# Acly/dlimgedit

Hardware: AMD Instinct MI355X
Metric: images/sec encode+mask @1024x1024 (higher is better)
Workload: dtype f16; 1 GPU; SAM vit_b encoder + 1 point prompt, 1 image(s)/GPU/step, 1024x1024 RGBA, inputs and masks resident in HBM; timed through the extension entry point dlimg_amd_encode_and_mask (device pointers in and out) -- the drop-in table itself, host buffers in and out, is `abi_path`; weights=seeded synthetic, lanes_per_gpu=4, lanes_fed_by_the_step_queue=3, requests_coalesced_per_pass=4, passes_queued_per_lane=2

## Files before the change

dlimgedit_amd/csrc/kernels/attention_window.hip:

```cpp
#include "device_common.hpp"
#include "kernels.hpp"

#include <algorithm>
#include <cstdio>
#include <cstdlib>
#include <mutex>
#include <string>
#include <vector>

namespace dlimg {
namespace {

constexpr int WS = 14;
constexpr int SLOTS = 224;
constexpr int NW = 5;
constexpr int GRID = 64;
constexpr int V_STRIDE = 96;
constexpr int G_STRIDE = 33;
typedef short short4_t __attribute__((ext_vector_type(4)));
typedef __attribute__((address_space(3))) short4_t lds_short4_t;

struct WinSlot { int token; bool dummy; bool pad; };

DLIMG_DEVICE WinSlot win_slot(int slot, int wy, int wx) {
    int ty = slot >> 4, tx = slot & 15;
    int gy = wy * WS + ty, gx = wx * WS + tx;
    WinSlot s;
    s.dummy = tx >= WS;
    s.pad = !s.dummy && (gy >= GRID || gx >= GRID);
    s.token = gy * GRID + gx;
    return s;
}

DLIMG_DEVICE int k_row(int slot) { const int tx = slot & 15; return (slot >> 4) * WS + (tx < WS ? tx : WS - 1); }

template <int HD>
__global__ __launch_bounds__(448, 4) void attention_window_kernel(const half_t* __restrict__ qkv,
                                                               const half_t* __restrict__ qkv_pad,
                                                               const half_t* __restrict__ rel_h,
                                                               const half_t* __restrict__ rel_w,
                                                               half_t* __restrict__ out, int heads,
                                                               unsigned long long* stamps_arg) {
#ifdef DLIMG_TUNING
    unsigned long long* const stamps = stamps_arg;
#else
    unsigned long long* const stamps = nullptr;
#endif
    unsigned long long tstamp[8] = {0, 0, 0, 0, 0, 0, 0, 0};
    auto stamp = [&](int i) { if (stamps) tstamp[i] = __builtin_amdgcn_s_memtime(); };
    stamp(0);
    constexpr int KS = HD / 16;
    constexpr int DT = (HD + 31) / 32;
    constexpr int K_STRIDE = HD + 8;
    constexpr int CHUNKS = HD / 8;
    static_assert(DT * 32 <= V_STRIDE, "head dimension tiles must fit the padded V row");

    extern __shared__ __attribute__((aligned(16))) char smem[];
    half_t* lds_k = reinterpret_cast<half_t*>(smem);
    half_t* lds_v = lds_k + WS * WS * K_STRIDE;
    float* lds_g = reinterpret_cast<float*>(smem);

    const int D = heads * HD;
    const int ld = 3 * D;
    const int head = blockIdx.x % heads;
    const int win = (blockIdx.x / heads) % (NW * NW);
    const int img = blockIdx.x / (heads * NW * NW);
    const int wy = win / NW, wx = win % NW;
    const half_t* base = qkv + (size_t)img * 4096 * ld;
    const int tid = threadIdx.x;
    const int lane = lane_id();
    const int wave = wave_id();
    const int hi = lane >> 5, l31 = lane & 31;

    const int token0 = wy * WS * GRID + wx * WS;
    const int qslot = wave * 32 + l31;
    const WinSlot qs = win_slot(qslot, wy, wx);
    const bool q_real = !qs.dummy && !qs.pad;
    half8_t qf[KS];
    {
        const half_t* qrow = base + (size_t)(q_real ? qs.token : token0) * ld + head * HD + hi * 8;
#pragma unroll
        for (int ks = 0; ks < KS; ++ks) qf[ks] = *reinterpret_cast<const half8_t*>(qrow + ks * 16);
    }
    half8_t rfh[KS], rfw[KS];
    {
        const int rrow = l31 < 2 * WS - 1 ? l31 : 2 * WS - 2;
#pragma unroll
        for (int ks = 0; ks < KS; ++ks) {
            rfh[ks] = *reinterpret_cast<const half8_t*>(rel_h + rrow * HD + ks * 16 + hi * 8);
            rfw[ks] = *reinterpret_cast<const half8_t*>(rel_w + rrow * HD + ks * 16 + hi * 8);
        }
    }
    static_assert((SLOTS * CHUNKS) % 448 == 0, "K/V chunks split evenly over the workgroup");
    constexpr int KV_IT = SLOTS * CHUNKS / 448;
#if defined(DLIMG_TUNING) && defined(DLIMG_WINDOW_KV_EARLY)
    constexpr int KV_EARLY = HD == 64 ? KV_IT : DLIMG_WINDOW_KV_EARLY;
#else
    constexpr int KV_EARLY = HD == 64 ? KV_IT : 3;
#endif
    half8_t kreg[KV_IT], vreg[KV_IT];
    auto request_kv = [&](int it) {
        const int idx = tid + it * 448;
        const WinSlot ws = win_slot(idx / CHUNKS, wy, wx);
        const half_t* row = (ws.pad ? qkv_pad : base + (size_t)(ws.dummy ? token0 : ws.token) * ld) + head * HD + (idx % CHUNKS) * 8;
        kreg[it] = *reinterpret_cast<const half8_t*>(row + D);
        vreg[it] = *reinterpret_cast<const half8_t*>(row + 2 * D);
    };
#pragma unroll
    for (int it = 0; it < KV_EARLY; ++it) request_kv(it);
    __builtin_amdgcn_sched_barrier(0);
    stamp(1);
#pragma unroll
    for (int ks = 0; ks < KS; ++ks) {
        if (!q_real) qf[ks] = zero_h8();
        if (l31 >= 2 * WS - 1) { rfh[ks] = zero_h8(); rfw[ks] = zero_h8(); }
    }

    float* g = lds_g + wave * 32 * G_STRIDE;
    const int ty_q = qslot >> 4, tx_q = qslot & 15;
    float bh[WS];
    float bw[8];
    {
        float16_t acc = zero16();
#pragma unroll
        for (int ks = 0; ks < KS; ++ks) acc = mfma32(rfh[ks], qf[ks], acc);
#pragma unroll
        for (int r = 0; r < 16; ++r) g[l31 * G_STRIDE + acc_row(r, hi)] = acc[r];
        __builtin_amdgcn_sched_barrier(0);
        float16_t acc_w = zero16();
#pragma unroll
        for (int ks = 0; ks < KS; ++ks) acc_w = mfma32(rfw[ks], qf[ks], acc_w);
        if (KV_EARLY < KV_IT) {
            __builtin_amdgcn_sched_barrier(0);
#pragma unroll
            for (int it = KV_EARLY; it < KV_IT; ++it) request_kv(it);
            __builtin_amdgcn_sched_barrier(0);
        }
        __builtin_amdgcn_fence(__ATOMIC_RELEASE, "wavefront");
        __builtin_amdgcn_wave_barrier();
#pragma unroll
        for (int ky = 0; ky < WS; ++ky) bh[ky] = g[l31 * G_STRIDE + ty_q + (WS - 1) - ky] * sqrtf((float)HD);
        __builtin_amdgcn_fence(__ATOMIC_RELEASE, "wavefront");
        __builtin_amdgcn_wave_barrier();
#pragma unroll
        for (int r = 0; r < 16; ++r) g[l31 * G_STRIDE + acc_row(r, hi)] = acc_w[r];
        __builtin_amdgcn_fence(__ATOMIC_RELEASE, "wavefront");
        __builtin_amdgcn_wave_barrier();
#pragma unroll
        for (int e = 0; e < 8; ++e) {
            const int tx = (e & 3) + 8 * (e >> 2) + 4 * hi;
            bw[e] = tx < WS ? g[l31 * G_STRIDE + tx_q + (WS - 1) - tx] * sqrtf((float)HD) : -INFINITY;
        }
        __syncthreads();
    }
    stamp(2);

#pragma unroll
    for (int it = 0; it < KV_IT; ++it) {
        const int idx = tid + it * 448;
        const int slot = idx / CHUNKS, ch = idx % CHUNKS;
        const bool dummy = (slot & 15) >= WS;
        if (!dummy) *reinterpret_cast<half8_t*>(lds_k + k_row(slot) * K_STRIDE + ch * 8) = kreg[it];
        *reinterpret_cast<half8_t*>(lds_v + slot * V_STRIDE + ch * 8) = dummy ? zero_h8() : vreg[it];
    }
    if (DT * 32 > HD) {
        constexpr int PADC = (DT * 32 - HD) / 8;
        for (int idx = tid; idx < SLOTS * PADC; idx += 448)
            *reinterpret_cast<half8_t*>(lds_v + (idx / PADC) * V_STRIDE + HD + (idx % PADC) * 8) = zero_h8();
    }
    __syncthreads();
    stamp(3);

    const float scale = rsqrtf((float)HD);

    const half_t* kb = lds_k + k_row(l31) * K_STRIDE + hi * 8;
    auto score_tile = [&](int jt) {
        float16_t t;
#pragma unroll
        for (int r = 0; r < 16; ++r) {
            const int ty = jt * 2 + (r >> 3);
            const int e = (r & 3) + 4 * ((r >> 2) & 1);
            t[r] = bh[ty] + bw[e];
        }
#pragma unroll
        for (int ks = 0; ks < KS; ++ks) {
            half8_t kf = *reinterpret_cast<const half8_t*>(kb + (jt * 2 * WS) * K_STRIDE + ks * 16);
            t = mfma32(kf, qf[ks], t);
        }
        return t;
    };
#if defined(DLIMG_TUNING) && defined(DLIMG_WINDOW_TWO_PASS)
    constexpr bool ONLINE = false;
#else
    constexpr bool ONLINE = true;
#endif
    constexpr bool TWO_PASS = HD == 64 && !ONLINE;
    float16_t kept[(TWO_PASS || ONLINE) ? 1 : 7];
    float m = -INFINITY;
    const float c = scale * 1.44269504088896341f;
    if (!ONLINE) {
#pragma unroll
        for (int jt = 0; jt < 7; ++jt) {
            const float16_t t = score_tile(jt);
            if (!TWO_PASS) kept[jt] = t;
#pragma unroll
            for (int r = 0; r < 16; ++r) m = fmaxf(m, t[r]);
            __builtin_amdgcn_sched_barrier(0);
        }
        m = fmaxf(m, swap_halves(m));
    }
    stamp(4);
    float mc = -m * c;
    if (TWO_PASS) {
#pragma unroll
        for (int i = 0; i < WS; ++i) asm volatile("" : "+v"(bh[i]));
#pragma unroll
        for (int i = 0; i < 8; ++i) asm volatile("" : "+v"(bw[i]));
    }

    const half_t* vb = lds_v + ((hi * 4 + ((lane & 15) >> 2)) * V_STRIDE) + 16 * ((lane >> 4) & 1) + 4 * (lane & 3);
    float16_t o[DT];
#pragma unroll
    for (int dt = 0; dt < DT; ++dt) o[dt] = zero16();
    float l = 0.f;
#pragma unroll
    for (int jt = 0; jt < 7; ++jt) {
        float16_t t = (TWO_PASS || ONLINE) ? score_tile(jt) : kept[(TWO_PASS || ONLINE) ? 0 : jt];
        if (ONLINE) {
            float tm = fmaxf(fmaxf(t[0], t[1]), t[2]);
#pragma unroll
            for (int r = 3; r < 15; r += 2) tm = fmaxf(fmaxf(tm, t[r]), t[r + 1]);
            tm = fmaxf(tm, t[15]);
            tm = fmaxf(tm, swap_halves(tm));
            if (jt == 0) {
                m = tm;
                mc = -m * c;
            } else if (__any(__builtin_fmaf(tm, c, mc) > 8.0f)) {
                const float m_new = fmaxf(m, tm);
                const float alpha = __builtin_amdgcn_exp2f((m - m_new) * c);
#pragma unroll
                for (int dt = 0; dt < DT; ++dt)
#pragma unroll
                    for (int r = 0; r < 16; ++r) o[dt][r] *= alpha;
                l *= alpha;
                m = m_new;
                mc = -m * c;
            }
        }
#pragma unroll
        for (int r = 0; r < 16; ++r) {
            const float pv = __builtin_amdgcn_exp2f(__builtin_fmaf(t[r], c, mc));
            t[r] = pv;
            l += pv;
        }
#pragma unroll
        for (int st = 0; st < 2; ++st) {
            half8_t pf;
#pragma unroll
            for (int e = 0; e < 8; ++e) pf[e] = (half_t)t[st * 8 + e];
            const int key0 = jt * 32 + st * 16;
#pragma unroll
            for (int dt = 0; dt < DT; ++dt) {
                const half_t* vp = vb + key0 * V_STRIDE + dt * 32;
                const short4_t v0 = __builtin_amdgcn_ds_read_tr16_b64_v4i16((lds_short4_t*)vp);
                const short4_t v1 = __builtin_amdgcn_ds_read_tr16_b64_v4i16((lds_short4_t*)(vp + 8 * V_STRIDE));
                const half4_t h0 = __builtin_bit_cast(half4_t, v0), h1 = __builtin_bit_cast(half4_t, v1);
                half8_t vf = {h0[0], h0[1], h0[2], h0[3], h1[0], h1[1], h1[2], h1[3]};
                o[dt] = mfma32(vf, pf, o[dt]);
            }
        }
        __builtin_amdgcn_sched_barrier(0);
    }
    l += swap_halves(l);
    const float inv_l = 1.0f / l;
    stamp(5);

    __syncthreads();
    stamp(6);
    constexpr int ROWB = HD * 2 + 16;
    static_assert(7 * 32 * ROWB <= WS * WS * K_STRIDE * 2 + SLOTS * V_STRIDE * 2, "output slabs must fit in the K / V images");
    char* slab = smem + wave * 32 * ROWB;
#pragma unroll
    for (int dt = 0; dt < DT; ++dt)
#pragma unroll
        for (int g4 = 0; g4 < 4; ++g4) {
            const int d0 = dt * 32 + 8 * g4;
            if (d0 < HD) {
                const half4_t v = {(half_t)(o[dt][g4 * 4 + 0] * inv_l), (half_t)(o[dt][g4 * 4 + 1] * inv_l),
                                   (half_t)(o[dt][g4 * 4 + 2] * inv_l), (half_t)(o[dt][g4 * 4 + 3] * inv_l)};
                *reinterpret_cast<half4_t*>(slab + l31 * ROWB + hi * 8 + d0 * 2) = v;
            }
        }
    asm volatile("s_waitcnt lgkmcnt(0)" ::: "memory");
    constexpr int NIT = (32 * CHUNKS + 63) / 64;
#pragma unroll
    for (int it = 0; it < NIT; ++it) {
        const int idx = it * 64 + lane;
        const int row = idx / CHUNKS, ch = idx % CHUNKS;
        if (row < 32) {
            const WinSlot os = win_slot(wave * 32 + row, wy, wx);
            if (!os.dummy && !os.pad) {
                const float4_t v = *reinterpret_cast<const float4_t*>(slab + row * ROWB + ch * 16);
                store16_result(out + ((size_t)img * 4096 + os.token) * D + head * HD + ch * 8, v);
            }
        }
    }
    if (stamps && tid == 0) {
        asm volatile("s_waitcnt vmcnt(0)" ::: "memory");
        tstamp[7] = __builtin_amdgcn_s_memtime();
#pragma unroll
        for (int i = 0; i < 8; ++i) stamps[(size_t)blockIdx.x * 8 + i] = tstamp[i];
    }
}

template <int HD>
void launch_window(const half_t* qkv, const half_t* bias, const half_t* rel_h, const half_t* rel_w, half_t* out, int B,
                   int heads, hipStream_t s) {
    const size_t images = (size_t)WS * WS * (HD + 8) * 2 + (size_t)SLOTS * V_STRIDE * 2;
    const size_t scratch = 7 * 32 * G_STRIDE * 4;
    const size_t lds = images > scratch ? images : scratch;
    static k::LdsOptIn opt_in;
    opt_in.ensure((const void*)attention_window_kernel<HD>, lds, "attention_window: the device refuses the kernel's LDS size");
    unsigned long long* stamps = nullptr;
#ifdef DLIMG_TUNING
    static const bool want = std::getenv("DLIMGEDIT_WINDOW_STAMPS") != nullptr;
    static unsigned long long* buf = nullptr;
    const int wgs = B * NW * NW * heads;
    if (want) {
        if (!buf) (void)hipMalloc(&buf, (size_t)64 * NW * NW * 64 * 8 * sizeof(unsigned long long));
        if (wgs <= 64 * NW * NW * 64) stamps = buf;
    }
#endif
    hipLaunchKernelGGL(attention_window_kernel<HD>, dim3(B * NW * NW * heads), dim3(448), lds, s, qkv, bias, rel_h,
                       rel_w, out, heads, stamps);
#ifdef DLIMG_TUNING
    if (stamps) {
        static int launches = 0;
        if (++launches % 50 == 0) {
            (void)hipStreamSynchronize(s);
            std::vector<unsigned long long> h((size_t)wgs * 8);
            (void)hipMemcpy(h.data(), stamps, h.size() * sizeof(unsigned long long), hipMemcpyDeviceToHost);
            static const char* names[7] = {"requests", "rel-pos", "K/V->LDS", "pass 1", "pass 2", "barrier", "store"};
            std::string line = "[window stamps] " + std::to_string(wgs) + " workgroups, median cycles:";
            for (int p = 0; p < 7; ++p) {
                std::vector<unsigned long long> d(wgs);
                for (int w = 0; w < wgs; ++w) d[w] = h[(size_t)w * 8 + p + 1] - h[(size_t)w * 8 + p];
                std::nth_element(d.begin(), d.begin() + wgs / 2, d.end());
                line += std::string(" ") + names[p] + " " + std::to_string(d[wgs / 2]);
            }
            std::vector<unsigned long long> d(wgs);
            unsigned long long t0 = ~0ull, t1 = 0;
            for (int w = 0; w < wgs; ++w) { d[w] = h[(size_t)w * 8 + 7] - h[(size_t)w * 8]; t0 = std::min(t0, h[(size_t)w * 8]); t1 = std::max(t1, h[(size_t)w * 8 + 7]); }
            std::nth_element(d.begin(), d.begin() + wgs / 2, d.end());
            line += " | whole " + std::to_string(d[wgs / 2]) + " | first start to last end " + std::to_string(t1 - t0);
            fprintf(stderr, "%s\n", line.c_str());
        }
    }
#endif
}

}

namespace k {

void attention_window(const half_t* qkv, const half_t* qkv_pad, const half_t* rel_h, const half_t* rel_w, half_t* out,
                      int B, int heads, int hd, hipStream_t s) {
    if (B <= 0 || heads <= 0) throw_error("attention_window: empty problem");
    if (((uintptr_t)qkv | (uintptr_t)out | (uintptr_t)qkv_pad | (uintptr_t)rel_h | (uintptr_t)rel_w) & 15)
        throw_error("attention_window: buffers must be 16-byte aligned");
    switch (hd) {
    case 64: return launch_window<64>(qkv, qkv_pad, rel_h, rel_w, out, B, heads, s);
    case 80: return launch_window<80>(qkv, qkv_pad, rel_h, rel_w, out, B, heads, s);
    default: throw_error("attention_window: head dimension must be 64 or 80");
    }
}

}
}
```

Before: 912.1 images/s.

## Pack window queries densely, skip dead waves, and fold rel-pos bias into softmax offsets

Queries are mapped densely over the real tokens of each window instead of a 16-wide slot grid, so edge windows leave whole waves with no queries. Those waves only help stage K/V into LDS and then exit early. The softmax now folds the row bias and the scale into per-row exp2 offsets exchanged with permlane32_swap. It optimistically exponentiates against a running reference and recomputes a tile only when sums overflow a threshold. This cuts MFMA and exp work in padded windows and removes the per-element bias add, at the cost of a more complex rescale path and extra barriers that the early-exit waves must match.

Result: no change. 913.5 images/s (median of 6 runs) (+0.2%).

```diff
diff --git a/dlimgedit_amd/csrc/kernels/attention_window.hip b/dlimgedit_amd/csrc/kernels/attention_window.hip
--- a/dlimgedit_amd/csrc/kernels/attention_window.hip
+++ b/dlimgedit_amd/csrc/kernels/attention_window.hip
@@ -30,6 +30,25 @@
     s.pad = !s.dummy && (gy >= GRID || gx >= GRID);
     s.token = gy * GRID + gx;
     return s;
+}
+
+struct WinQuery { int ty, tx, token; bool real; };
+
+DLIMG_DEVICE WinQuery win_query(int pos, int wy, int wx) {
+    const int rows = wy == NW - 1 ? GRID - (NW - 1) * WS : WS;
+    const bool narrow = wx == NW - 1;
+    const int cols = narrow ? GRID - (NW - 1) * WS : WS;
+    static_assert(GRID - (NW - 1) * WS == 8, "the narrow window's row is a shift");
+    WinQuery q;
+    q.real = pos < rows * cols;
+    q.ty = q.real ? (narrow ? pos >> 3 : pos / WS) : 0;
+    q.tx = q.real ? (narrow ? pos & 7 : pos % WS) : 0;
+    q.token = (wy * WS + q.ty) * GRID + wx * WS + q.tx;
+    return q;
+}
+
+DLIMG_DEVICE int win_queries(int wy, int wx) {
+    return (wy == NW - 1 ? GRID - (NW - 1) * WS : WS) * (wx == NW - 1 ? GRID - (NW - 1) * WS : WS);
 }
 
 DLIMG_DEVICE int k_row(int slot) { const int tx = slot & 15; return (slot >> 4) * WS + (tx < WS ? tx : WS - 1); }
@@ -73,24 +92,9 @@
     const int hi = lane >> 5, l31 = lane & 31;
 
     const int token0 = wy * WS * GRID + wx * WS;
-    const int qslot = wave * 32 + l31;
-    const WinSlot qs = win_slot(qslot, wy, wx);
-    const bool q_real = !qs.dummy && !qs.pad;
-    half8_t qf[KS];
-    {
-        const half_t* qrow = base + (size_t)(q_real ? qs.token : token0) * ld + head * HD + hi * 8;
-#pragma unroll
-        for (int ks = 0; ks < KS; ++ks) qf[ks] = *reinterpret_cast<const half8_t*>(qrow + ks * 16);
-    }
-    half8_t rfh[KS], rfw[KS];
-    {
-        const int rrow = l31 < 2 * WS - 1 ? l31 : 2 * WS - 2;
-#pragma unroll
-        for (int ks = 0; ks < KS; ++ks) {
-            rfh[ks] = *reinterpret_cast<const half8_t*>(rel_h + rrow * HD + ks * 16 + hi * 8);
-            rfw[ks] = *reinterpret_cast<const half8_t*>(rel_w + rrow * HD + ks * 16 + hi * 8);
-        }
-    }
+    const WinQuery qs = win_query(wave * 32 + l31, wy, wx);
+    const bool q_real = qs.real;
+    const bool wave_live = wave * 32 < win_queries(wy, wx);
     static_assert((SLOTS * CHUNKS) % 448 == 0, "K/V chunks split evenly over the workgroup");
     constexpr int KV_IT = SLOTS * CHUNKS / 448;
 #if defined(DLIMG_TUNING) && defined(DLIMG_WINDOW_KV_EARLY)
@@ -106,6 +110,45 @@
         kreg[it] = *reinterpret_cast<const half8_t*>(row + D);
         vreg[it] = *reinterpret_cast<const half8_t*>(row + 2 * D);
     };
+    auto kv_to_lds = [&]() {
+#pragma unroll
+        for (int it = 0; it < KV_IT; ++it) {
+            const int idx = tid + it * 448;
+            const int slot = idx / CHUNKS, ch = idx % CHUNKS;
+            const bool dummy = (slot & 15) >= WS;
+            if (!dummy) *reinterpret_cast<half8_t*>(lds_k + k_row(slot) * K_STRIDE + ch * 8) = kreg[it];
+            *reinterpret_cast<half8_t*>(lds_v + slot * V_STRIDE + ch * 8) = dummy ? zero_h8() : vreg[it];
+        }
+        if (DT * 32 > HD) {
+            constexpr int PADC = (DT * 32 - HD) / 8;
+            for (int idx = tid; idx < SLOTS * PADC; idx += 448)
+                *reinterpret_cast<half8_t*>(lds_v + (idx / PADC) * V_STRIDE + HD + (idx % PADC) * 8) = zero_h8();
+        }
+    };
+    if (!wave_live) {
+#pragma unroll
+        for (int it = 0; it < KV_IT; ++it) request_kv(it);
+        __syncthreads();
+        kv_to_lds();
+        __syncthreads();
+        __syncthreads();
+        return;
+    }
+    half8_t qf[KS];
+    {
+        const half_t* qrow = base + (size_t)(q_real ? qs.token : token0) * ld + head * HD + hi * 8;
+#pragma unroll
+        for (int ks = 0; ks < KS; ++ks) qf[ks] = *reinterpret_cast<const half8_t*>(qrow + ks * 16);
+    }
+    half8_t rfh[KS], rfw[KS];
+    {
+        const int rrow = l31 < 2 * WS - 1 ? l31 : 2 * WS - 2;
+#pragma unroll
+        for (int ks = 0; ks < KS; ++ks) {
+            rfh[ks] = *reinterpret_cast<const half8_t*>(rel_h + rrow * HD + ks * 16 + hi * 8);
+            rfw[ks] = *reinterpret_cast<const half8_t*>(rel_w + rrow * HD + ks * 16 + hi * 8);
+        }
+    }
 #pragma unroll
     for (int it = 0; it < KV_EARLY; ++it) request_kv(it);
     __builtin_amdgcn_sched_barrier(0);
@@ -117,9 +160,10 @@
     }
 
     float* g = lds_g + wave * 32 * G_STRIDE;
-    const int ty_q = qslot >> 4, tx_q = qslot & 15;
-    float bh[WS];
-    float bw[8];
+    const int ty_q = qs.ty, tx_q = qs.tx;
+    const float c = rsqrtf((float)HD) * 1.44269504088896341f;
+    float bhc[WS / 2];
+    float bw8[8];
     {
         float16_t acc = zero16();
 #pragma unroll
@@ -139,7 +183,8 @@
         __builtin_amdgcn_fence(__ATOMIC_RELEASE, "wavefront");
         __builtin_amdgcn_wave_barrier();
 #pragma unroll
-        for (int ky = 0; ky < WS; ++ky) bh[ky] = g[l31 * G_STRIDE + ty_q + (WS - 1) - ky] * sqrtf((float)HD);
+        for (int jt = 0; jt < WS / 2; ++jt)
+            bhc[jt] = g[l31 * G_STRIDE + ty_q + (WS - 1) - (2 * jt + hi)] * sqrtf((float)HD) * c;
         __builtin_amdgcn_fence(__ATOMIC_RELEASE, "wavefront");
         __builtin_amdgcn_wave_barrier();
 #pragma unroll
@@ -149,39 +194,22 @@
 #pragma unroll
         for (int e = 0; e < 8; ++e) {
             const int tx = (e & 3) + 8 * (e >> 2) + 4 * hi;
-            bw[e] = tx < WS ? g[l31 * G_STRIDE + tx_q + (WS - 1) - tx] * sqrtf((float)HD) : -INFINITY;
-        }
-        __syncthreads();
-    }
+            bw8[e] = tx < WS ? g[l31 * G_STRIDE + tx_q + (WS - 1) - tx] * sqrtf((float)HD) : -INFINITY;
+        }
+    }
+    __syncthreads();
     stamp(2);
 
-#pragma unroll
-    for (int it = 0; it < KV_IT; ++it) {
-        const int idx = tid + it * 448;
-        const int slot = idx / CHUNKS, ch = idx % CHUNKS;
-        const bool dummy = (slot & 15) >= WS;
-        if (!dummy) *reinterpret_cast<half8_t*>(lds_k + k_row(slot) * K_STRIDE + ch * 8) = kreg[it];
-        *reinterpret_cast<half8_t*>(lds_v + slot * V_STRIDE + ch * 8) = dummy ? zero_h8() : vreg[it];
-    }
-    if (DT * 32 > HD) {
-        constexpr int PADC = (DT * 32 - HD) / 8;
-        for (int idx = tid; idx < SLOTS * PADC; idx += 448)
-            *reinterpret_cast<half8_t*>(lds_v + (idx / PADC) * V_STRIDE + HD + (idx % PADC) * 8) = zero_h8();
-    }
+    kv_to_lds();
     __syncthreads();
     stamp(3);
 
-    const float scale = rsqrtf((float)HD);
-
+    float16_t bw;
+#pragma unroll
+    for (int r = 0; r < 16; ++r) bw[r] = bw8[r & 7];
     const half_t* kb = lds_k + k_row(l31) * K_STRIDE + hi * 8;
-    auto score_tile = [&](int jt) {
-        float16_t t;
-#pragma unroll
-        for (int r = 0; r < 16; ++r) {
-            const int ty = jt * 2 + (r >> 3);
-            const int e = (r & 3) + 4 * ((r >> 2) & 1);
-            t[r] = bh[ty] + bw[e];
-        }
+    auto score_tile = [&](int jt, const half_t* kb) {
+        float16_t t = bw;
 #pragma unroll
         for (int ks = 0; ks < KS; ++ks) {
             half8_t kf = *reinterpret_cast<const half8_t*>(kb + (jt * 2 * WS) * K_STRIDE + ks * 16);
@@ -189,119 +217,126 @@
         }
         return t;
     };
-#if defined(DLIMG_TUNING) && defined(DLIMG_WINDOW_TWO_PASS)
-    constexpr bool ONLINE = false;
-#else
-    constexpr bool ONLINE = true;
-#endif
-    constexpr bool TWO_PASS = HD == 64 && !ONLINE;
-    float16_t kept[(TWO_PASS || ONLINE) ? 1 : 7];
-    float m = -INFINITY;
-    const float c = scale * 1.44269504088896341f;
-    if (!ONLINE) {
-#pragma unroll
-        for (int jt = 0; jt < 7; ++jt) {
-            const float16_t t = score_tile(jt);
-            if (!TWO_PASS) kept[jt] = t;
-#pragma unroll
-            for (int r = 0; r < 16; ++r) m = fmaxf(m, t[r]);
-            __builtin_amdgcn_sched_barrier(0);
-        }
-        m = fmaxf(m, swap_halves(m));
-    }
+    auto expo = [&](const float16_t& t, float off0, float off1, half8_t (&pf)[2]) {
+        float ps[2] = {0.f, 0.f};
+#pragma unroll
+        for (int r = 0; r < 16; ++r) {
+            const float pv = __builtin_amdgcn_exp2f(__builtin_fmaf(t[r], c, r < 8 ? off0 : off1));
+            ps[r & 1] += pv;
+            pf[r >> 3][r & 7] = (half_t)pv;
+        }
+        return ps[0] + ps[1];
+    };
+    auto tile_max = [&](const float16_t& t, float off0, float off1) {
+        float a = fmaxf(fmaxf(t[0], t[1]), t[2]), b = fmaxf(fmaxf(t[8], t[9]), t[10]);
+#pragma unroll
+        for (int r = 3; r < 7; r += 2) {
+            a = fmaxf(fmaxf(a, t[r]), t[r + 1]);
+            b = fmaxf(fmaxf(b, t[r + 8]), t[r + 9]);
+        }
+        a = fmaxf(a, t[7]);
+        b = fmaxf(b, t[15]);
+        const float e = fmaxf(__builtin_fmaf(a, c, off0), __builtin_fmaf(b, c, off1));
+        return fmaxf(e, swap_halves(e));
+    };
     stamp(4);
-    float mc = -m * c;
-    if (TWO_PASS) {
-#pragma unroll
-        for (int i = 0; i < WS; ++i) asm volatile("" : "+v"(bh[i]));
-#pragma unroll
-        for (int i = 0; i < 8; ++i) asm volatile("" : "+v"(bw[i]));
-    }
 
     const half_t* vb = lds_v + ((hi * 4 + ((lane & 15) >> 2)) * V_STRIDE) + 16 * ((lane >> 4) & 1) + 4 * (lane & 3);
     float16_t o[DT];
-#pragma unroll
-    for (int dt = 0; dt < DT; ++dt) o[dt] = zero16();
-    float l = 0.f;
-#pragma unroll
-    for (int jt = 0; jt < 7; ++jt) {
-        float16_t t = (TWO_PASS || ONLINE) ? score_tile(jt) : kept[(TWO_PASS || ONLINE) ? 0 : jt];
-        if (ONLINE) {
-            float tm = fmaxf(fmaxf(t[0], t[1]), t[2]);
-#pragma unroll
-            for (int r = 3; r < 15; r += 2) tm = fmaxf(fmaxf(tm, t[r]), t[r + 1]);
-            tm = fmaxf(tm, t[15]);
-            tm = fmaxf(tm, swap_halves(tm));
-            if (jt == 0) {
-                m = tm;
-                mc = -m * c;
-            } else if (__any(__builtin_fmaf(tm, c, mc) > 8.0f)) {
-                const float m_new = fmaxf(m, tm);
-                const float alpha = __builtin_amdgcn_exp2f((m - m_new) * c);
-#pragma unroll
-                for (int dt = 0; dt < DT; ++dt)
-#pragma unroll
-                    for (int r = 0; r < 16; ++r) o[dt][r] *= alpha;
-                l *= alpha;
-                m = m_new;
-                mc = -m * c;
-            }
-        }
-#pragma unroll
-        for (int r = 0; r < 16; ++r) {
-            const float pv = __builtin_amdgcn_exp2f(__builtin_fmaf(t[r], c, mc));
-            t[r] = pv;
-            l += pv;
-        }
-#pragma unroll
-        for (int st = 0; st < 2; ++st) {
-            half8_t pf;
-#pragma unroll
-            for (int e = 0; e < 8; ++e) pf[e] = (half_t)t[st * 8 + e];
-            const int key0 = jt * 32 + st * 16;
-#pragma unroll
-            for (int dt = 0; dt < DT; ++dt) {
-                const half_t* vp = vb + key0 * V_STRIDE + dt * 32;
-                const short4_t v0 = __builtin_amdgcn_ds_read_tr16_b64_v4i16((lds_short4_t*)vp);
-                const short4_t v1 = __builtin_amdgcn_ds_read_tr16_b64_v4i16((lds_short4_t*)(vp + 8 * V_STRIDE));
-                const half4_t h0 = __builtin_bit_cast(half4_t, v0), h1 = __builtin_bit_cast(half4_t, v1);
-                half8_t vf = {h0[0], h0[1], h0[2], h0[3], h1[0], h1[1], h1[2], h1[3]};
-                o[dt] = mfma32(vf, pf, o[dt]);
-            }
-        }
-        __builtin_amdgcn_sched_barrier(0);
-    }
-    l += swap_halves(l);
-    const float inv_l = 1.0f / l;
+    float inv_l;
+    {
+#pragma unroll
+        for (int dt = 0; dt < DT; ++dt) o[dt] = zero16();
+        float l = 0.f;
+        float mref = 0.f;
+#pragma unroll
+        for (int jt = 0; jt < 7; ++jt) {
+            float off0, off1;
+            auto row_addends = [&]() {
+                const unsigned mine = __builtin_bit_cast(unsigned, bhc[jt] - mref);
+                const auto both = __builtin_amdgcn_permlane32_swap(mine, mine, false, false);
+                const unsigned lower = both[0], upper = both[1];
+                off0 = __builtin_bit_cast(float, lower);
+                off1 = __builtin_bit_cast(float, upper);
+            };
+            half8_t pf[2];
+            float ts = 0.f;
+            if (jt > 0) {
+                row_addends();
+                ts = expo(score_tile(jt, kb), off0, off1, pf);
+            }
+            if (jt == 0 || __any(!(ts <= 256.f))) {
+                const half_t* kb_again = kb;
+                if (jt > 0) asm volatile("" : "+v"(kb_again));
+                const float16_t t = score_tile(jt, kb_again);
+                if (jt == 0) row_addends();
+                const float d = tile_max(t, off0, off1);
+                if (jt > 0) {
+                    const float m_new = mref + fmaxf(d, 0.f);
+                    const float alpha = __builtin_amdgcn_exp2f(mref - m_new);
+#pragma unroll
+                    for (int dt = 0; dt < DT; ++dt)
+#pragma unroll
+                        for (int r = 0; r < 16; ++r) o[dt][r] *= alpha;
+                    l *= alpha;
+                    mref = m_new;
+                } else {
+                    mref = d;
+                }
+                row_addends();
+                ts = expo(t, off0, off1, pf);
+            }
+
+            l += ts;
+#pragma unroll
+            for (int st = 0; st < 2; ++st) {
+                const int key0 = jt * 32 + st * 16;
+#pragma unroll
+                for (int dt = 0; dt < DT; ++dt) {
+                    const half_t* vp = vb + key0 * V_STRIDE + dt * 32;
+                    const short4_t v0 = __builtin_amdgcn_ds_read_tr16_b64_v4i16((lds_short4_t*)vp);
+                    const short4_t v1 = __builtin_amdgcn_ds_read_tr16_b64_v4i16((lds_short4_t*)(vp + 8 * V_STRIDE));
+                    const half4_t h0 = __builtin_bit_cast(half4_t, v0), h1 = __builtin_bit_cast(half4_t, v1);
+                    half8_t vf = {h0[0], h0[1], h0[2], h0[3], h1[0], h1[1], h1[2], h1[3]};
+                    o[dt] = mfma32(vf, pf[st], o[dt]);
+                }
+            }
+            __builtin_amdgcn_sched_barrier(0);
+        }
+        l += swap_halves(l);
+        inv_l = 1.0f / l;
+    }
     stamp(5);
 
     __syncthreads();
     stamp(6);
     constexpr int ROWB = HD * 2 + 16;
     static_assert(7 * 32 * ROWB <= WS * WS * K_STRIDE * 2 + SLOTS * V_STRIDE * 2, "output slabs must fit in the K / V images");
-    char* slab = smem + wave * 32 * ROWB;
-#pragma unroll
-    for (int dt = 0; dt < DT; ++dt)
-#pragma unroll
-        for (int g4 = 0; g4 < 4; ++g4) {
-            const int d0 = dt * 32 + 8 * g4;
-            if (d0 < HD) {
-                const half4_t v = {(half_t)(o[dt][g4 * 4 + 0] * inv_l), (half_t)(o[dt][g4 * 4 + 1] * inv_l),
-                                   (half_t)(o[dt][g4 * 4 + 2] * inv_l), (half_t)(o[dt][g4 * 4 + 3] * inv_l)};
-                *reinterpret_cast<half4_t*>(slab + l31 * ROWB + hi * 8 + d0 * 2) = v;
-            }
-        }
-    asm volatile("s_waitcnt lgkmcnt(0)" ::: "memory");
-    constexpr int NIT = (32 * CHUNKS + 63) / 64;
-#pragma unroll
-    for (int it = 0; it < NIT; ++it) {
-        const int idx = it * 64 + lane;
-        const int row = idx / CHUNKS, ch = idx % CHUNKS;
-        if (row < 32) {
-            const WinSlot os = win_slot(wave * 32 + row, wy, wx);
-            if (!os.dummy && !os.pad) {
-                const float4_t v = *reinterpret_cast<const float4_t*>(slab + row * ROWB + ch * 16);
-                store16_result(out + ((size_t)img * 4096 + os.token) * D + head * HD + ch * 8, v);
+    {
+        char* slab = smem + wave * 32 * ROWB;
+#pragma unroll
+        for (int dt = 0; dt < DT; ++dt)
+#pragma unroll
+            for (int g4 = 0; g4 < 4; ++g4) {
+                const int d0 = dt * 32 + 8 * g4;
+                if (d0 < HD) {
+                    const half4_t v = {(half_t)(o[dt][g4 * 4 + 0] * inv_l), (half_t)(o[dt][g4 * 4 + 1] * inv_l),
+                                       (half_t)(o[dt][g4 * 4 + 2] * inv_l), (half_t)(o[dt][g4 * 4 + 3] * inv_l)};
+                    *reinterpret_cast<half4_t*>(slab + l31 * ROWB + hi * 8 + d0 * 2) = v;
+                }
+            }
+        asm volatile("s_waitcnt lgkmcnt(0)" ::: "memory");
+        constexpr int NIT = (32 * CHUNKS + 63) / 64;
+#pragma unroll
+        for (int it = 0; it < NIT; ++it) {
+            const int idx = it * 64 + (int)__builtin_amdgcn_mbcnt_hi(~0u, __builtin_amdgcn_mbcnt_lo(~0u, 0u));
+            const int row = idx / CHUNKS, ch = idx % CHUNKS;
+            if (row < 32) {
+                const WinQuery os = win_query(wave * 32 + row, wy, wx);
+                if (os.real) {
+                    const float4_t v = *reinterpret_cast<const float4_t*>(slab + row * ROWB + ch * 16);
+                    store16_result(out + ((size_t)img * 4096 + os.token) * D + head * HD + ch * 8, v);
+                }
             }
         }
     }
@@ -340,7 +375,7 @@
             (void)hipStreamSynchronize(s);
             std::vector<unsigned long long> h((size_t)wgs * 8);
             (void)hipMemcpy(h.data(), stamps, h.size() * sizeof(unsigned long long), hipMemcpyDeviceToHost);
-            static const char* names[7] = {"requests", "rel-pos", "K/V->LDS", "pass 1", "pass 2", "barrier", "store"};
+            static const char* names[7] = {"requests", "rel-pos", "K/V->LDS", "setup", "softmax pass", "barrier", "store"};
             std::string line = "[window stamps] " + std::to_string(wgs) + " workgroups, median cycles:";
             for (int p = 0; p < 7; ++p) {
                 std::vector<unsigned long long> d(wgs);
```
